# mkln/spamtree

Measured on AMD Instinct MI355X. Metric: Gibbs iterations/sec + achieved HBM GB/s, n=1e6 grid, 1/2/4/8 MI355X, higher is better.
Workload: dtype f64

## Files before the change

### spamtree_amd/csrc/spamtree_fit.cpp

```cpp
#include "spamtree_fit.h"

#include <chrono>
#include <cmath>
#include <cstdlib>
#include <cstring>
#include <string>
#include <vector>

namespace {

struct HostRng {
  uint32_t k0, k1;
  explicit HostRng(uint64_t seed) : k0((uint32_t)seed), k1((uint32_t)(seed >> 32)) {}
  void block(uint32_t c0, uint32_t c1, uint32_t c2, uint32_t c3, uint32_t out[4]) const {
    uint32_t a = k0, b = k1;
    for (int r = 0; r < 10; ++r) {
      const uint64_t p0 = 0xD2511F53ull * c0, p1 = 0xCD9E8D57ull * c2;
      const uint32_t n0 = (uint32_t)(p1 >> 32) ^ c1 ^ a, n2 = (uint32_t)(p0 >> 32) ^ c3 ^ b;
      c1 = (uint32_t)p1; c3 = (uint32_t)p0; c0 = n0; c2 = n2;
      a += 0x9E3779B9u; b += 0xBB67AE85u;
    }
    out[0] = c0; out[1] = c1; out[2] = c2; out[3] = c3;
  }
  static double u01(uint32_t a, uint32_t b) {
// ... 174 lines not shown

extern "C" int stm_init(stm_chain c) {
  if (!c || !c->h) return ST_ERR_USAGE;
  if (c->initialised) return ST_OK;
  for (int slot = 0; slot < 2; ++slot) {
    const int rc = st_factor(c->h, slot, c->param.data(), c->k, &c->loglik[slot]);
    if (rc < 0) { c->err = st_last_error(c->h); return rc; }
    if (rc > 0) { c->err = "starting theta is not positive definite"; return ST_ERR_USAGE; }
  }
  c->current_loglik = c->loglik[0];
  c->initialised = true;
  return ST_OK;
}

static int draw_tausq_beta(stm_chain c);
static int step_w_theta(stm_chain c, bool early_ok = true) {
  const uint32_t m = (uint32_t)c->m;
  int rc;
  const int k = c->k;
  RAMAdapt &am = c->am;
  std::vector<double> U(k), np(k);
  if (c->sample_theta) {
    am.count_proposal();
    for (int i = 0; i < k; ++i) U[i] = c->rng.normal(i, 0, m, 1);
    for (int j = 0; j < k; ++j) {
      double f = logit(c->param[j], c->bounds[j], c->bounds[k + j]);
      for (int i = 0; i < k; ++i) f += am.paramsd[(size_t)i * k + j] * U[i];
      np[j] = logistic(f, c->bounds[j], c->bounds[k + j]);
    }
    for (int j = 0; j < k; ++j) {
      if (np[j] < c->bounds[j]) np[j] = c->bounds[j] + 1e-10;
// ... 14 lines not shown
  };
  if (c->sample_w) {
    rc = st_sample_w_loglik_begin(c->h, nullptr, c->seed, m, 0);
    if (rc) { c->err = st_last_error(c->h); return rc; }
    if ((!c->sample_theta || !c->defer_sync) && (rc = finish_sweep()) != 0) return rc;
    sweep_open = c->sample_theta && c->defer_sync;
  }
  if (c->sample_theta) {
    c->theta_alt = np;
    double new_ll = c->loglik[1];
    if (c->early_beta && early_ok && c->sample_w && st_factor_is_async(c->h)) {
      rc = st_factor_enqueue(c->h, 1, np.data(), k);
      if (rc == 0) {
        const int r3 = draw_tausq_beta(c);
        c->tb_drawn = true;
        rc = st_factor_finish(c->h, &new_ll);
        if (r3) return r3;
      }
    } else
    rc = st_factor(c->h, 1, np.data(), k, &new_ll);
    if (sweep_open) {
      const int r2 = finish_sweep();
      if (r2) return r2;
    }
    if (rc < 0) { c->err = st_last_error(c->h); return rc; }
    const bool acceptable = rc == 0;
    if (acceptable) c->loglik[1] = new_ll;
    c->current_loglik = c->loglik[0];
    if (std::isnan(c->current_loglik)) { c->err = "At nan loglik: error."; return STM_ERR_NAN; }
    double jac = 0;
// ... 54 lines not shown
    if ((rc = st_set_beta(c->h, c->Bcoeff.data())) != 0) { c->err = st_last_error(c->h); return rc; }
  }
  return ST_OK;
}
static int step_tausq_beta(stm_chain c) {
  if (!c->tb_drawn) { const int rc = draw_tausq_beta(c); if (rc) return rc; }
  c->tb_drawn = false;
  c->m += 1;
  return ST_OK;
}

extern "C" int stm_step(stm_chain c, int n_iters) {
  if (!c || !c->h) return ST_ERR_USAGE;
  if (!c->initialised) { const int rc0 = stm_init(c); if (rc0) return rc0; }
  for (int it = 0; it < n_iters; ++it) {
    int rc = step_w_theta(c);
    if (rc) return rc;
    rc = step_tausq_beta(c);
    if (rc) return rc;
  }
  return ST_OK;
}

extern "C" int stm_state(stm_chain c, double *theta, double *Bcoeff, double *tausq_inv, double *loglik, double *accept_ratio,
                         int64_t *iteration, double *paramsd) {
  if (!c) return ST_ERR_USAGE;
  if (theta) std::memcpy(theta, c->param.data(), c->param.size() * sizeof(double));
  if (Bcoeff) std::memcpy(Bcoeff, c->Bcoeff.data(), c->Bcoeff.size() * sizeof(double));
  if (tausq_inv) std::memcpy(tausq_inv, c->tausq_inv.data(), c->tausq_inv.size() * sizeof(double));
  if (loglik) *loglik = c->current_loglik;
  if (accept_ratio) *accept_ratio = c->am.accept_ratio;
// ... 114 lines not shown
```

### spamtree_amd/csrc/spamtree_hip.hip

```cpp

#include "st_device.hpp"
#include "factor_generic.hpp"
#include "factor_mfma.hpp"
#include "chol_blocked.hpp"
#include "factor_quad.hpp"
#include "factor_big.hpp"
#include "factor_wide.hpp"
#include "factor_lchain.hpp"
#include "sample_kernels.hpp"
#include "misc_kernels.hpp"
#include "predict_points.hpp"
#include "simulate_kernels.hpp"

static thread_local std::string g_create_error;
struct st_handle_s;
static void points_free(st_handle_s *h);

template <typename T>
struct DevBuf {
  T *p = nullptr;
  size_t n = 0;
  hipError_t alloc(size_t count) {
    n = count;
    if (count == 0) { p = nullptr; return hipSuccess; }
// ... 59 lines not shown
  "k_factor_mfma", "k_factor_lchain<96>", "k_factor_lchain<136>", "k_factor_ref_finish", "k_lchain_scalars", "k_factor_wide<WG_JT>",
  "k_factor_bigmfma<3, 5, 34>", "k_factor_bigmfma<4, 5, 34>", "k_factor_bigmfma<5, 3, 24>",
  "k_gram", "k_gram_direct", "k_gram_big",
  "k_sample_mfma", "k_sample_leaf_seg<4>", "k_sample_leaf_seg<6>", "k_sample_leaf", "k_sample_wave", "k_sample_lean<true>",
  "k_sample_lean<false>", "k_sample<true, false>", "k_sample_leaf_wide", "k_sample<true, true>", "k_sample<false>",
};

struct Switches {
  int wide = 1, split_gram = 1, sample_wave = 1;
  bool lchain = true, lchain_ref = true, gram_big = true, gram_direct = true, sample_lean = true, sample_lat = true,
       leaf_seg = true, leaf_wide = true, async_top = true;
  int lchain_ref_min = 1;
  int factor_gen = 3;
  int quad_units = 0;
  int quad_min = -1;
};

static Switches read_switches() {
  auto level = [](const char *name) {
    const char *e = getenv(name);
    return (e && e[0] == '0') ? 0 : ((e && e[0] == '2') ? 2 : 1);
  };
  Switches s;
  s.wide = level("SPAMTREE_WIDE"); s.split_gram = level("SPAMTREE_SPLIT_GRAM"); s.sample_wave = level("SPAMTREE_SAMPLE_WAVE");
  s.lchain = level("SPAMTREE_LCHAIN"); s.lchain_ref = level("SPAMTREE_LCHAIN_REF"); s.gram_big = level("SPAMTREE_GRAM_BIG");
  s.gram_direct = level("SPAMTREE_GRAM_DIRECT"); s.sample_lean = level("SPAMTREE_SAMPLE_LEAN"); s.sample_lat = level("SPAMTREE_SAMPLE_LAT");
  s.leaf_seg = level("SPAMTREE_LEAF_SEG"); s.leaf_wide = level("SPAMTREE_LEAF_WIDE"); s.async_top = level("SPAMTREE_ASYNC_TOP");
  const char *e;
  if ((e = getenv("SPAMTREE_LCHAIN_REF_MIN"))) s.lchain_ref_min = atoi(e);
  if ((e = getenv("SPAMTREE_FACTOR_KERNEL")) && e[0] == '1') s.factor_gen = 1;
  if ((e = getenv("SPAMTREE_QUAD_UNITS"))) s.quad_units = atoi(e);
  if ((e = getenv("SPAMTREE_QUAD_MIN"))) s.quad_min = std::max(atoi(e), 0);
  return s;
}

struct st_handle_s {
  std::string err;
  int device = 0;
  hipStream_t stream = nullptr;
  int quirks = 1, force_generic = 0;
  Switches sw;
  long long n_all = 0, n_blocks = 0;
  int q = 1, p = 1, d = 2, n_groups = 0, n_actual_groups = 0;
  long long n_obs = 0;
  size_t lds_limit = 65536;
  int sm_count = 256;

// ... 28 lines not shown
  DevBuf<int> d_ownobs;
  std::vector<int> own_grp_list, own_obs_slow;
  DevBuf<int> d_owngrp, d_ownslow;
  DevBuf<unsigned char> d_rowmask, d_blkmask;
  DevBuf<double> d_comm;
  DevBuf<double> d_gather;
  DevBuf<int> d_gidx;
  int gather_cnt = 1;
  DevBuf<double> d_gerr;
  hipStream_t stream2 = nullptr;
  hipEvent_t ev_top = nullptr, ev_main = nullptr;
  DevBuf<int> d_err2, d_toplist;
  int n_toplist = 0, g_top = 0;
  bool async_top = false, top_pending = false, prof_suspend = false, async_top_off = false;
  hipEvent_t ev_stats = nullptr;
  bool stats_on_stream2 = false;
  bool stats_prefetched = false;
  int top_phys = -1;
  std::vector<double> top_theta;
  long long top_off = 0, top_len = 0;
  std::vector<std::pair<long long, long long>> top_zero;
  bool ext_stream = false;
  DevBuf<double> d_sum_w, d_sum_yhat;
  long long n_summary = 0;
  DevBuf<double> d_draws_w, d_draws_yhat;
  long long draws_cap = 0, n_draws = 0;
  int gram_direct_level = -1;
  bool stats_valid = false;
  bool host_stats_valid = false;
  std::vector<double> host_stats;
  double *pin = nullptr;
  double *pin_up = nullptr;
  int pin_up_slot = 0, pin_up_len = 0;
  hipEvent_t ev_up[2] = {nullptr, nullptr};
  bool factor_open = false; int factor_open_slot = 0;
  std::vector<double> top_theta_open;
  hipEvent_t ev_factor = nullptr;
  std::vector<char> s0_valid;
  bool gram_valid = false;
  bool cache_gram = true;
  bool defer_leaf = false;
  bool leaf_pending[2] = {false, false};
  CovPar leaf_cp[2];
  DevBuf<double> d_vleaf;
  bool limited = false;
  std::vector<int> twin_list;
  DevBuf<int> d_twin;
  int twin_maxM = 1;
  ncclComm_t comm = nullptr;
  std::vector<LevelInfo> levels;
  std::vector<int> route_a, route_b;
  int route_p = R_NONE;
// ... 9 lines not shown
  std::vector<SimLevel> sim_levels;

  DevBuf<double> d_cx, d_cy, d_y, d_X, d_w, d_xb, d_z, d_B, d_panels[2], d_acc, d_logdet[2], d_loglik[2], d_scalars, d_partial,
      d_stats, d_scratch, d_tmp_n, d_tsq;
  DevBuf<int> d_mv, d_anc, d_dch, d_lvl, d_pred, d_allobs, d_err;
  DevBuf<unsigned char> d_obs;
  DevBuf<long long> d_dev2model, d_partner;
  DevBuf<Blk> d_blks;
  size_t panel_total = 0, acc_total = 0;
  long long scratch_stride = 0;
  int scratch_wgs = 0;
  int slot_map[2] = {0, 1};
  double tausq_inv[QMAX];
  std::vector<double> theta[2];
  bool z_valid = false;

  int prof = 0;
  double prof_ms[ST_N_KERNEL_FAMILIES] = {0};
  long long prof_n[ST_N_KERNEL_FAMILIES] = {0};
  std::vector<double> prof_level_ms;
  std::vector<long long> prof_level_n;
  struct ProfRec { hipEvent_t a, b; int fam, level, count; };
  std::vector<ProfRec> prof_pending;
  std::vector<hipEvent_t> ev_free;
};

#define HCHK(h, call)                                                                                         \
  do {                                                                                                        \
    hipError_t e_ = (call);                                                                                   \
    if (e_ != hipSuccess) {                                                                                   \
// ... 77 lines not shown
extern "C" void st_set_create_error(const char *msg) { g_create_error = msg ? msg : ""; }

extern "C" int st_destroy(st_handle h) {
  if (!h) return ST_OK;
  (void)hipSetDevice(h->device);
  h->d_cx.free(); h->d_cy.free(); h->d_y.free(); h->d_X.free(); h->d_w.free(); h->d_xb.free(); h->d_z.free(); h->d_B.free();
  h->d_panels[0].free(); h->d_panels[1].free(); h->d_acc.free();
  for (int s = 0; s < 2; ++s) { h->d_logdet[s].free(); h->d_loglik[s].free(); }
  h->d_scalars.free(); h->d_partial.free(); h->d_stats.free(); h->d_scratch.free(); h->d_tmp_n.free(); h->d_tsq.free();
  h->d_mv.free(); h->d_anc.free(); h->d_dch.free(); h->d_lvl.free(); h->d_pred.free(); h->d_allobs.free(); h->d_err.free();
  h->d_twin.free(); h->d_wgrps.free(); h->d_lcslabs.free(); h->d_lcrow.free(); h->d_rfvoff.free(); h->d_vscr.free(); h->d_vleaf.free(); h->d_s0.free(); h->d_s0off.free(); h->d_obs.free(); h->d_dev2model.free(); h->d_partner.free(); h->d_blks.free(); h->d_grps.free(); h->d_quads.free(); h->d_gdesc.free();
  h->d_ownobs.free(); h->d_owngrp.free(); h->d_ownslow.free(); h->d_rowmask.free(); h->d_blkmask.free(); h->d_comm.free(); h->d_gather.free(); h->d_gidx.free(); h->d_gerr.free(); h->d_err2.free(); h->d_toplist.free();
  if (h->ev_top) (void)hipEventDestroy(h->ev_top);
  if (h->ev_main) (void)hipEventDestroy(h->ev_main);
  if (h->ev_stats) (void)hipEventDestroy(h->ev_stats);
  if (h->stream2) (void)hipStreamDestroy(h->stream2); h->d_sum_w.free(); h->d_sum_yhat.free(); h->d_draws_w.free(); h->d_draws_yhat.free();
  prof_harvest(h);
  for (auto e : h->ev_free) (void)hipEventDestroy(e);
  if (h->comm) (void)ncclCommDestroy(h->comm);
  if (h->pin) (void)hipHostFree(h->pin);
  if (h->pin_up) (void)hipHostFree(h->pin_up);
  for (int i = 0; i < 2; ++i) if (h->ev_up[i]) (void)hipEventDestroy(h->ev_up[i]);
  if (h->ev_factor) (void)hipEventDestroy(h->ev_factor);
  points_free(h);
  h->d_simz.free(); h->d_sime.free(); h->d_simw.free(); h->d_simy.free(); h->d_rowblk.free();
  if (h->stream && !h->ext_stream) (void)hipStreamDestroy(h->stream);
  delete h;
  return ST_OK;
}

static int create_impl(const st_problem *pb, const st_options *opt, st_handle *out, bool plan_only, int64_t *owner_out, int32_t *cut_out);

extern "C" int st_create(const st_problem *pb, const st_options *opt, st_handle *out) {
  return create_impl(pb, opt, out, false, nullptr, nullptr);
}

extern "C" int st_shard_plan(const st_problem *pb, int32_t world, int64_t *owner, int32_t *cut_level) {
  st_options opt = {0, 1, 0, world, 0, 0};
// ... 628 lines not shown
      for (int b2 = 0; b2 < pb->p; ++b2)
        h->xtx[(size_t)v * pb->p * pb->p + (size_t)b2 * pb->p + a] += pb->X[(size_t)a * n + r] * pb->X[(size_t)b2 * n + r];
  }

#define CCHK(call)                                                                                            \
  do {                                                                                                        \
    hipError_t e_ = (call);                                                                                   \
    if (e_ != hipSuccess) return fail_create(h, ST_ERR_HIP, std::string(#call) + ": " + hipGetErrorString(e_)); \
  } while (0)
  CCHK(hipStreamCreate(&h->stream));
  CCHK(hipHostMalloc((void **)&h->pin, 64 * sizeof(double), hipHostMallocDefault));
  h->pin_up_len = QMAX + std::max(1, h->p * h->q);
  CCHK(hipHostMalloc((void **)&h->pin_up, (size_t)2 * h->pin_up_len * sizeof(double), hipHostMallocDefault));
  for (int i = 0; i < 2; ++i) CCHK(hipEventCreateWithFlags(&h->ev_up[i], hipEventDisableTiming));
  CCHK(hipEventCreateWithFlags(&h->ev_factor, hipEventDisableTiming));
  CCHK(h->d_cx.upload(cx)); CCHK(h->d_cy.upload(cy)); CCHK(h->d_y.upload(y)); CCHK(h->d_X.upload(X));
  CCHK(h->d_mv.upload(mv)); CCHK(h->d_obs.upload(obs)); CCHK(h->d_partner.upload(partner));
  CCHK(h->d_dev2model.upload(h->dev2model));
  {
    std::vector<Blk> db = h->blks;
    if (h->limited) for (Blk &B : db) B.acc_len = 0;
    CCHK(h->d_blks.upload(db));
    if (h->limited) { std::vector<int> t = h->twin_list; if (t.empty()) t.push_back(0); CCHK(h->d_twin.upload(t)); }
  }
  { std::vector<int> a = h->anc_idx; if (a.empty()) a.push_back(0); CCHK(h->d_anc.upload(a)); }
  { std::vector<int> a = h->dch_idx; if (a.empty()) a.push_back(0); CCHK(h->d_dch.upload(a)); }
  CCHK(h->d_lvl.upload(h->lvl_list));
  { std::vector<Grp> g = h->grps; if (g.empty()) g.push_back(Grp{0, 0, 0, 0, 0}); CCHK(h->d_grps.upload(g)); }
  {
    int stride = 8;
// ... 214 lines not shown
  {
    h->g_top = 0;
    bool all_fast = !h->limited && !h->force_generic;
    for (int g = 0; g < n_actual; ++g) all_fast = all_fast && h->levels[g].fast;
    if (all_fast) {
      while (h->g_top < n_actual && !(h->sw.factor_gen == 3 && h->levels[h->g_top].q_nkx > 0)) ++h->g_top;
      if (h->g_top >= n_actual) h->g_top = 0;
    }
    h->async_top = h->g_top > 0 && h->sw.async_top;
    std::vector<int> tl;
    for (int b : h->own_obs_list) if (h->blks[b].level < h->g_top) tl.push_back(b);
    h->n_toplist = (int)tl.size();
    if (tl.empty()) tl.push_back(0);
    CCHK(h->d_toplist.upload(tl));
    CCHK(h->d_err2.alloc(2));
    if (h->async_top) {
      CCHK(hipStreamCreateWithFlags(&h->stream2, hipStreamNonBlocking));
      CCHK(hipEventCreateWithFlags(&h->ev_top, hipEventDisableTiming));
      CCHK(hipEventCreateWithFlags(&h->ev_main, hipEventDisableTiming));
      CCHK(hipEventCreateWithFlags(&h->ev_stats, hipEventDisableTiming));
    }
  }
  (void)hipGetLastError();
#undef CCHK
  h->s0_valid.assign((size_t)std::max(n_actual, 1), 0);
  h->prof_level_ms.assign(2 * n_actual, 0.0);
  h->prof_level_n.assign(2 * n_actual, 0);
  *out = h;
  return ST_OK;
}

static int upload_rows(st_handle h, const double *src, double *dst) {
  std::vector<double> tmp(h->n_all);
  for (long long i = 0; i < h->n_all; ++i) tmp[i] = src[h->dev2model[i]];
  HCHK(h, hipMemcpyAsync(dst, tmp.data(), h->n_all * sizeof(double), hipMemcpyHostToDevice, h->stream));
// ... 12 lines not shown
  if (!h || !w) return ST_ERR_USAGE;
  invalidate_stats(h);
  HCHK(h, hipSetDevice(h->device));
  return upload_rows(h, w, h->d_w.p);
}
extern "C" int st_get_w(st_handle h, double *w) {
  if (!h || !w) return ST_ERR_USAGE;
  HCHK(h, hipSetDevice(h->device));
  return download_rows(h, h->d_w.p, w);
}
extern "C" int st_get_xb(st_handle h, double *xb) {
  if (!h || !xb) return ST_ERR_USAGE;
  HCHK(h, hipSetDevice(h->device));
  return download_rows(h, h->d_xb.p, xb);
}
extern "C" int st_set_beta(st_handle h, const double *Bcoeff) {
  if (!h || !Bcoeff) return ST_ERR_USAGE;
  invalidate_stats(h);
  HCHK(h, hipSetDevice(h->device));
  h->pin_up_slot ^= 1;
  HCHK(h, hipEventSynchronize(h->ev_up[h->pin_up_slot]));
  double *stg = h->pin_up + (size_t)h->pin_up_slot * h->pin_up_len + QMAX;
  std::memcpy(stg, Bcoeff, (size_t)h->p * h->q * sizeof(double));
  HCHK(h, hipMemcpyAsync(h->d_B.p, stg, (size_t)h->p * h->q * sizeof(double), hipMemcpyHostToDevice, h->stream));
  HCHK(h, hipEventRecord(h->ev_up[h->pin_up_slot], h->stream));
  {
    ProfScope ps(h, 4);
    const int grid = (int)((h->n_all + NT - 1) / NT);
    hipLaunchKernelGGL(k_xb, dim3(grid), dim3(NT), 0, h->stream, h->d_X.p, h->d_mv.p, h->d_B.p, h->n_all, h->p, h->d_xb.p);
  }
  HCHK(h, hipGetLastError());
  return ST_OK;
}
extern "C" int st_set_tausq_inv(st_handle h, const double *t) {
  if (!h || !t) return ST_ERR_USAGE;
  for (int j = 0; j < h->q; ++j) h->tausq_inv[j] = t[j];
  HCHK(h, hipSetDevice(h->device));
  h->pin_up_slot ^= 1;
  HCHK(h, hipEventSynchronize(h->ev_up[h->pin_up_slot]));
  double *stg = h->pin_up + (size_t)h->pin_up_slot * h->pin_up_len;
  std::memcpy(stg, h->tausq_inv, QMAX * sizeof(double));
  HCHK(h, hipMemcpyAsync(h->d_tsq.p, stg, QMAX * sizeof(double), hipMemcpyHostToDevice, h->stream));
  HCHK(h, hipEventRecord(h->ev_up[h->pin_up_slot], h->stream));
  return ST_OK;
}
static int settle_top(st_handle h) {
  if (h->top_pending) { HCHK(h, hipSetDevice(h->device)); HCHK(h, hipStreamWaitEvent(h->stream, h->ev_top, 0)); }
  return ST_OK;
}
static int complete_leaf(st_handle h, int slot) {
  const int phys = h->slot_map[slot];
  if (!h->leaf_pending[phys]) return ST_OK;
  HCHK(h, hipSetDevice(h->device));
  const CovPar &cp = h->leaf_cp[phys];
  ProfScope phase(h, 0, -2, 0);
  for (int g = 0; g < h->n_actual_groups; ++g) {
    const LevelInfo &L = h->levels[g];
    if (L.vl_off < 0) continue;
    QuadArgs F;
    std::memset(&F, 0, sizeof(F));
    F.blks = h->d_blks.p; F.anc_idx = h->d_anc.p; F.grps = h->d_grps.p + L.grp_first;
    F.quads = h->d_quads.p + L.quad_first + L.qown_lo; F.nquad = L.qown_n;
// ... 202 lines not shown
        hipLaunchKernelGGL((k_factor_wide<WG_JT>), dim3(std::min(L.wide_count, h->sm_count)), dim3(WG_NT), L.lds_wide, st, W, cp);
      } else if (L.bigmfma && h->sw.factor_gen == 3) {
        A.scratch = h->d_scratch.p; A.scratch_stride = h->scratch_stride; A.SR = L.bm_ldS;
        if (L.maxM <= 48) { route(g, R_BIGMFMA3); hipLaunchKernelGGL((k_factor_bigmfma<3, 5, 34>), dim3(std::min(A.nlist, h->sm_count)), dim3(BM_NT), L.lds_bigmfma, st, A, cp); }
        else if (L.maxM <= 64) { route(g, R_BIGMFMA4); hipLaunchKernelGGL((k_factor_bigmfma<4, 5, 34>), dim3(std::min(A.nlist, h->sm_count)), dim3(BM_NT), L.lds_bigmfma, st, A, cp); }
        else { route(g, R_BIGMFMA5); hipLaunchKernelGGL((k_factor_bigmfma<5, 3, 24>), dim3(std::min(A.nlist, h->sm_count)), dim3(BM_NT), L.lds_bigmfma, st, A, cp); }
      } else if (L.big_factor) { route(g, R_FACTOR_SCRATCH); launch_factor<true, MODE_FACTOR>(h, L, A, cp, st); }
      else { route(g, R_FACTOR_LDS); launch_factor<false, MODE_FACTOR>(h, L, A, cp, st); }
    }
    HCHK(h, hipGetLastError());
  }
  return ST_OK;
}


extern "C" int st_factor_ahead_levels(st_handle h) { return (h && h->async_top && !h->async_top_off) ? h->g_top : 0; }
extern "C" int st_factor_ahead_enable(st_handle h, int enable) {
  if (!h) return ST_ERR_USAGE;
  h->async_top_off = !enable;
  return ST_OK;
}
extern "C" int st_factor_begin(st_handle h, int slot, const double *theta, int ntheta) {
  if (!h || !theta || slot < 0 || slot > 1) return ST_ERR_USAGE;
  if (!h->async_top || h->async_top_off) return ST_OK;
  HCHK(h, hipSetDevice(h->device));
  CovPar cp;
  int rc = make_covpar(h, theta, ntheta, &cp);
  if (rc) return rc;
  if (h->top_pending) HCHK(h, hipStreamWaitEvent(h->stream2, h->ev_top, 0));
  HCHK(h, hipEventRecord(h->ev_main, h->stream));
  HCHK(h, hipStreamWaitEvent(h->stream2, h->ev_main, 0));
  const int init[2] = {INT_MAX, 0};
  HCHK(h, hipMemcpyAsync(h->d_err2.p, init, 2 * sizeof(int), hipMemcpyHostToDevice, h->stream2));
  const int phys = h->slot_map[slot];
  h->leaf_pending[phys] = false;
  h->prof_suspend = true;
  rc = factor_launch(h, phys, cp, 0, h->g_top, h->stream2, h->d_err2.p);
  h->prof_suspend = false;
  if (rc) return rc;
  HCHK(h, hipEventRecord(h->ev_top, h->stream2));
  h->top_pending = true; h->top_phys = phys; h->top_theta.assign(theta, theta + ntheta);
  return ST_OK;
}
static int fix_top_comps(st_handle h, int phys);
static int run_stats(st_handle h, hipStream_t st);
static int stats_begin(st_handle h) {
  if (!h->stream2 || h->stats_valid) return ST_OK;
  HCHK(h, hipEventRecord(h->ev_main, h->stream));
  HCHK(h, hipStreamWaitEvent(h->stream2, h->ev_main, 0));
  int rc = run_stats(h, h->stream2);
  if (rc) return rc;
  const size_t nq = (size_t)h->p * h->q + h->q;
  h->stats_prefetched = nq <= 40;
  if (h->stats_prefetched) HCHK(h, hipMemcpyAsync(h->pin + 20, h->d_stats.p, nq * sizeof(double), hipMemcpyDeviceToHost, h->stream2));
  HCHK(h, hipEventRecord(h->ev_stats, h->stream2));
  h->stats_on_stream2 = true;
  return ST_OK;
}

static int factor_local(st_handle h, int slot, const double *theta, int ntheta, bool vonly);
extern "C" int st_factor_local(st_handle h, int slot, const double *theta, int ntheta) { return factor_local(h, slot, theta, ntheta, false); }
static int factor_local(st_handle h, int slot, const double *theta, int ntheta, bool vonly) {
  if (!h || !theta || slot < 0 || slot > 1) return ST_ERR_USAGE;
  HCHK(h, hipSetDevice(h->device));
  CovPar cp;
  int rc = make_covpar(h, theta, ntheta, &cp);
  if (rc) return rc;
  h->theta[slot].assign(theta, theta + ntheta);
  if (slot == 0) { h->gram_valid = false; std::fill(h->s0_valid.begin(), h->s0_valid.end(), 0); }
  rc = reset_err(h);
  if (rc) return rc;
  const int phys = h->slot_map[slot];
  h->leaf_pending[phys] = false;
  if (slot == 1) { rc = stats_begin(h); if (rc) return rc; }
  bool reuse = false;
  if (h->top_pending) {
    HCHK(h, hipStreamWaitEvent(h->stream, h->ev_top, 0));
    reuse = h->top_phys == phys && (int)h->top_theta.size() == ntheta && std::equal(theta, theta + ntheta, h->top_theta.begin());
    h->top_pending = false;
  }
  bool deferred = false;
  rc = factor_launch(h, phys, cp, reuse ? h->g_top : 0, INT_MAX, nullptr, nullptr, vonly, &deferred);
  if (deferred) { h->leaf_pending[phys] = true; h->leaf_cp[phys] = cp; }
  if (rc || !reuse) return rc;
  rc = fix_top_comps(h, phys);
  if (rc) return rc;
  hipLaunchKernelGGL(k_merge_err, dim3(1), dim3(64), 0, h->stream, h->d_err.p, h->d_err2.p);
  HCHK(h, hipGetLastError());
  return ST_OK;
}

extern "C" int st_mg_pack_comps(st_handle h, int slot, void **dev_ptr, int64_t *len) {
  if (!h || slot < 0 || slot > 1) return ST_ERR_USAGE;
  HCHK(h, hipSetDevice(h->device));
  { const int rc0 = settle_top(h); if (rc0) return rc0; }
  const int phys = h->slot_map[slot], nb = (int)h->n_blocks;
  {
    ProfScope ps(h, 3);
    hipLaunchKernelGGL(k_pack_comps, dim3((std::max(nb, h->world) + NT - 1) / NT), dim3(NT), 0, h->stream, h->d_logdet[phys].p,
                       h->d_loglik[phys].p, h->d_blkmask.p, nb, h->d_err.p, h->rank, h->world, h->d_comm.p);
  }
// ... 69 lines not shown
  int rc = factor_enqueue(h, slot, theta, ntheta, false);
  if (rc) return rc;
  return st_factor_finish(h, loglik);
}
extern "C" int st_factor_is_async(st_handle h) { return (h && !(h->world > 1 || h->comm)) ? 1 : 0; }
extern "C" int st_factor_enqueue(st_handle h, int slot, const double *theta, int ntheta) {
  return factor_enqueue(h, slot, theta, ntheta, h && h->defer_leaf && slot == 1);
}
static int factor_enqueue(st_handle h, int slot, const double *theta, int ntheta, bool vonly) {
  if (!h || !theta || slot < 0 || slot > 1) return ST_ERR_USAGE;
  if (h->factor_open) { h->err = "st_factor_enqueue: the previous one has not been finished"; return ST_ERR_USAGE; }
  if (h->world > 1 || h->comm) {
    h->factor_open = true; h->factor_open_slot = slot; h->top_theta_open.assign(theta, theta + ntheta);
    return ST_OK;
  }
  int rc = factor_local(h, slot, theta, ntheta, vonly);
  if (rc) return rc;
  {
    ProfScope ps(h, 3);
    const int phys = h->slot_map[slot];
    launch_sum2(h->stream, h->d_logdet[phys].p, h->d_loglik[phys].p, (int)h->n_blocks, h->d_scalars.p + 8, h->d_scalars.p);
  }
  HCHK(h, hipGetLastError());
  HCHK(h, hipMemcpyAsync(h->pin + 12, h->d_scalars.p, 2 * sizeof(double), hipMemcpyDeviceToHost, h->stream));
  HCHK(h, hipMemcpyAsync(h->pin + 14, h->d_err.p, 2 * sizeof(int), hipMemcpyDeviceToHost, h->stream));
  HCHK(h, hipEventRecord(h->ev_factor, h->stream));
  h->factor_open = true; h->factor_open_slot = slot; h->top_theta_open.clear();
  return ST_OK;
}
extern "C" int st_factor_finish(st_handle h, double *loglik) {
  if (!h) return ST_ERR_USAGE;
  if (!h->factor_open) { h->err = "st_factor_finish without st_factor_enqueue"; return ST_ERR_USAGE; }
  h->factor_open = false;
  if (h->world > 1 || h->comm) {
    if (!h->comm) { h->err = "world > 1: call st_comm_init first, or use st_factor_local / st_mg_pack_comps / (all-reduce) / st_mg_finish"; return ST_ERR_USAGE; }
    int rc = st_factor_local(h, h->factor_open_slot, h->top_theta_open.data(), (int)h->top_theta_open.size());
    if (rc) return rc;
    return exchange_comps_and_finish(h, h->factor_open_slot, loglik);
  }
  HCHK(h, hipSetDevice(h->device));
  HCHK(h, hipEventSynchronize(h->ev_factor));
  const int e0 = ((const int *)(h->pin + 14))[0];
  if (e0 != INT_MAX) return e0 & 15;
  if (loglik) *loglik = h->pin[12] + h->pin[13];
  return ST_OK;
}

static int gather_w_scatter(st_handle h);
extern "C" int st_sample_w_loglik(st_handle h, const double *z, uint64_t seed, uint32_t iter, int slot, double *loglik) {
  if (!h || slot < 0 || slot > 1) return ST_ERR_USAGE;
  { const int rc0 = complete_leaf(h, slot); if (rc0) return rc0; }
  if (h->world > 1 || h->comm) {
    if (!h->comm) {
      int rc = st_sample_w(h, z, seed, iter);
      if (rc) return rc;
// ... 78 lines not shown
  }
  int rc = st_sample_w_local(h, z, seed, iter);
  if (rc) return rc;
  rc = st_sample_w_top(h);
  if (rc) return rc;
  HCHK(h, hipMemcpyAsync(h->pin + 10, h->d_err.p, 2 * sizeof(int), hipMemcpyDeviceToHost, h->stream));
  rc = st_loglik_local(h, slot);
  if (rc) return rc;
  {
    ProfScope ps(h, 3);
    const int phys = h->slot_map[slot];
    launch_sum2(h->stream, h->d_logdet[phys].p, h->d_loglik[phys].p, (int)h->n_blocks, h->d_scalars.p + 8, h->d_scalars.p);
  }
  HCHK(h, hipGetLastError());
  HCHK(h, hipMemcpyAsync(h->pin + 8, h->d_scalars.p, 2 * sizeof(double), hipMemcpyDeviceToHost, h->stream));
  h->c_rc = INT_MIN;
  h->c_pending = true;
  return ST_OK;
}
extern "C" int st_sample_w_loglik_end(st_handle h, double *loglik) {
  if (!h || !h->c_pending) return ST_ERR_USAGE;
  h->c_pending = false;
  if (h->c_rc != INT_MIN) {
    if (h->c_rc == ST_OK && loglik) *loglik = h->c_ll;
    return h->c_rc;
  }
  HCHK(h, hipStreamSynchronize(h->stream));
  const int e0 = ((const int *)(h->pin + 10))[0];
  if (e0 != INT_MAX) return e0 & 15;
  if (loglik) *loglik = h->pin[8] + h->pin[9];
  return ST_OK;
}

static int gen_or_upload_z(st_handle h, const double *z, uint64_t seed, uint32_t iter, unsigned stream_id, double *dst) {
  if (z) return upload_rows(h, z, dst);
  {
    ProfScope ps(h, 5);
    const int grid = (int)((h->n_all + NT - 1) / NT);
    hipLaunchKernelGGL(k_normals, dim3(grid), dim3(NT), 0, h->stream, dst, h->d_dev2model.p, h->n_all, iter, stream_id,
                       (unsigned long long)seed);
  }
  HCHK(h, hipGetLastError());
  return ST_OK;
}

static int sample_launch(st_handle h, int g_hi, int g_lo) {
  const int phys = h->slot_map[0];
  for (int g = g_hi - 1; g >= g_lo; --g) {
    const LevelInfo &L = h->levels[g];
    int *route = h->route_b.data() + 2 * (size_t)g;
    route[0] = route[1] = R_NONE;
    if ((L.fast ? L.gown_n : L.own_n) == 0) continue;
    SampleArgs A;
    std::memset(&A, 0, sizeof(A));
    A.blks = h->d_blks.p; A.anc_idx = h->d_anc.p; A.dch_idx = h->d_dch.p; A.list = h->d_lvl.p + L.first + L.own_lo; A.nlist = L.own_n;
    A.panels = h->d_panels[phys].p; A.w = h->d_w.p; A.y = h->d_y.p; A.xb = h->d_xb.p; A.z = h->d_z.p; A.mv = h->d_mv.p;
    A.obs = h->d_obs.p; A.acc = h->d_acc.p; A.errflag = h->d_err.p; A.maxP = L.maxP; A.maxM = L.maxM; A.maxLd = L.maxLd;
    for (int j = 0; j < QMAX; ++j) A.tausq_inv[j] = h->tausq_inv[j];
    A.do_gram = (h->gram_valid && h->cache_gram) ? 0 : 1;
    A.no_fwd = h->limited ? 1 : 0;
    A.lds_sq = (L.big_sample && L.sample_sq) ? 2 : 0;
    A.s0 = h->d_s0.p; A.s0off = h->d_s0off.p;
    {
// ... 58 lines not shown
        }
        if (L.big_sample) {
          A.scratch = h->d_scratch.p; A.scratch_stride = h->scratch_stride;
          if (L.isref) { route[1] = R_SAMPLE_BIG_REF; hipLaunchKernelGGL((k_sample<true, false>), dim3(std::min(L.own_n, h->scratch_wgs)), dim3(NT), L.lds_sample, h->stream, A); }
          else if (h->sw.leaf_wide && !A.do_gram && L.maxM <= 64 && L.maxMa <= 96 && L.maxJ <= 8) {
            route[1] = R_SAMPLE_LEAF_WIDE;
            hipLaunchKernelGGL(k_sample_leaf_wide, dim3(std::min(L.own_n, 16 * h->sm_count)), dim3(NT), ((size_t)4 * 64 * 12 + 3 * 64) * 8, h->stream, A);
          } else { route[1] = R_SAMPLE_BIG_LEAF; hipLaunchKernelGGL((k_sample<true, true>), dim3(std::min(L.own_n, h->scratch_wgs)), dim3(NT), L.lds_sample, h->stream, A); }
        } else {
          route[1] = R_SAMPLE_SMALL;
          hipLaunchKernelGGL((k_sample<false>), dim3(L.own_n), dim3(NT), L.lds_sample, h->stream, A);
        }
      }
    }
    HCHK(h, hipGetLastError());
  }
  return ST_OK;
}

extern "C" int st_sample_w_local(st_handle h, const double *z, uint64_t seed, uint32_t iter) {
  if (!h) return ST_ERR_USAGE;
  invalidate_stats(h);
  HCHK(h, hipSetDevice(h->device));
  int rc = gen_or_upload_z(h, z, seed, iter, 0u, h->d_z.p);
  if (rc) return rc;
  h->z_valid = true;
  rc = reset_err(h);
  if (rc) return rc;
  rc = sample_launch(h, h->n_actual_groups, std::min(h->cut, h->n_actual_groups));
  if (rc) return rc;
  for (auto &zr : h->top_zero) HCHK(h, hipMemsetAsync(h->d_acc.p + zr.first, 0, (size_t)zr.second * sizeof(double), h->stream));
  return ST_OK;
}
extern "C" int st_mg_top_region(st_handle h, void **dev_ptr, int64_t *len) {
  if (!h) return ST_ERR_USAGE;
  if (dev_ptr) *dev_ptr = h->d_acc.p + h->top_off;
  if (len) *len = h->top_len;
  return ST_OK;
}
extern "C" int st_sample_w_top(st_handle h) {
  if (!h) return ST_ERR_USAGE;
  invalidate_stats(h);
  HCHK(h, hipSetDevice(h->device));
  const int rc = sample_launch(h, std::min(h->cut, h->n_actual_groups), 0);
// ... 115 lines not shown
  }
  HCHK(h, hipGetLastError());
  HCHK(h, reset_err(h) == ST_OK ? hipSuccess : hipErrorUnknown);
  return ST_OK;
}
static int fix_top_comps(st_handle h, int phys) {
  if (h->n_toplist == 0) return ST_OK;
  int maxP = 0, maxM = 0;
  for (int g = 0; g < h->g_top; ++g) { maxP = std::max(maxP, h->levels[g].maxP); maxM = std::max(maxM, h->levels[g].maxM); }
  LoglikArgs A;
  A.blks = h->d_blks.p; A.anc_idx = h->d_anc.p; A.list = h->d_toplist.p; A.nlist = h->n_toplist;
  A.panels = h->d_panels[phys].p; A.w = h->d_w.p; A.loglik_c = h->d_loglik[phys].p; A.maxP = maxP; A.maxM = maxM;
  {
    ProfScope ps(h, 0, h->g_top > 0 ? h->g_top - 1 : 0);
    hipLaunchKernelGGL(k_loglik, dim3(A.nlist), dim3(NT), lds_loglik_bytes(maxP, maxM), h->stream, A);
  }
  HCHK(h, hipGetLastError());
  return ST_OK;
}
extern "C" int st_loglik_w(st_handle h, int slot, double *loglik) {
  if (!h) return ST_ERR_USAGE;
  if (slot >= 0 && slot <= 1) { const int rc0 = complete_leaf(h, slot); if (rc0) return rc0; }
  if (h->world > 1 || h->comm) {
    if (!h->comm) { h->err = "world > 1: call st_comm_init first, or use st_loglik_local / st_mg_pack_comps / (all-reduce) / st_mg_finish"; return ST_ERR_USAGE; }
    int rc = st_loglik_local(h, slot);
    if (rc) return rc;
    return exchange_comps_and_finish(h, slot, loglik);
  }
  int rc = st_loglik_local(h, slot);
  if (rc) return rc;
// ... 807 lines not shown
```

Baseline: 241.6.

## Overlap mid-level factorization on a low-priority stream and prefetch next normals

Extends the async top-level factor path so that the middle reference levels are factored on a third low-priority stream, launched during the sampling sweep after a gate level, with a separate loglik fixup kernel for those groups. The top-level factor launch is deferred until the sampling sweep has started, beta/tau uploads move to the side stream while a factor is open, the next iteration's normals are generated early, and a full stream sync is replaced by an event sync. The aim is to fill idle GPU time between the sweep tail and the factor, at the cost of more streams and events, more complex ordering, and possible contention with the sampling kernels.

```diff
diff --git a/profiles/r05/gaps.py b/profiles/r05/gaps.py
--- /dev/null
+++ b/profiles/r05/gaps.py
@@ -0,0 +1,79 @@
+import argparse
+import csv
+import json
+import statistics
+import sys
+
+
+def load(path):
+    rows = []
+    with open(path, newline="") as f:
+        for r in csv.DictReader(f):
+            rows.append((int(r["Start_Timestamp"]), int(r["End_Timestamp"]), r["Kernel_Name"],
+                         r.get("Queue_Id", "") + "/" + r.get("Stream_Id", "")))
+    rows.sort()
+    return rows
+
+
+def busy_ns(rows, t0, t1):
+    total, cur = 0, t0
+    for s, e, _, _ in rows:
+        if e <= t0 or s >= t1:
+            continue
+        s, e = max(s, cur), min(e, t1)
+        if e > s:
+            total += e - s
+            cur = e
+    return total
+
+
+def main():
+    ap = argparse.ArgumentParser()
+    ap.add_argument("trace")
+    ap.add_argument("--iters", type=int, default=20)
+    ap.add_argument("--gate", type=int, default=2)
+    args = ap.parse_args()
+    rows = load(args.trace)
+    starts = [i for i, r in enumerate(rows) if "k_normals" in r[2]]
+    tails, gaps = [], []
+    for a, b in zip(starts[:-1], starts[1:]):
+        it = rows[a:b]
+        main_q = it[0][3]
+        smp = [r for r in it if "k_sample" in r[2]]
+        llk = [r for r in it if "k_loglik_grp" in r[2]]
+        mrg = [r for r in it if "k_merge_err" in r[2]]
+        if len(smp) <= args.gate or not llk or not mrg:
+            continue
+        t0, t1 = smp[args.gate][1], llk[0][0]
+        other = sum(min(e, t1) - max(s, t0) for s, e, _, q in it if q != main_q and e > t0 and s < t1)
+        tails.append((t1 - t0, busy_ns(rows, t0, t1), other, sum(r[1] - r[0] for r in smp[args.gate + 1:])))
+        quad = [r for r in it if "k_factor_quad" in r[2] and r[0] < mrg[0][0]]
+        nxt = [r for r in rows[b:b + 40] if "k_sample" in r[2]]
+        if not quad or not nxt:
+            continue
+        g0, g1 = quad[-1][1], nxt[0][0]
+        inside = [r for r in rows[a:b + 40] if r[1] > g0 and r[0] < g1]
+        gaps.append((g1 - g0, busy_ns(rows, g0, g1), len(inside), sum(r[1] - r[0] for r in inside)))
+    tails, gaps = tails[-args.iters:], gaps[-args.iters:]
+
+    def med(xs, i):
+        return round(statistics.median(x[i] for x in xs) / 1e3, 1) if xs else None
+
+    span = [rows[s][0] for s in starts][-args.iters - 1:]
+    out = {
+        "iterations": len(tails),
+        "iteration_us": round(statistics.median(b - a for a, b in zip(span[:-1], span[1:])) / 1e3, 1) if len(span) > 1 else None,
+        "tail": {"wall_us": med(tails, 0), "busy_us": med(tails, 1), "idle_us": med(tails, 0) - med(tails, 1) if tails else None,
+                 "other_stream_us": med(tails, 2), "sweep_kernels_us": med(tails, 3)},
+        "gap": {"wall_us": med(gaps, 0), "busy_us": med(gaps, 1), "idle_us": med(gaps, 0) - med(gaps, 1) if gaps else None,
+                "kernels": med(gaps, 2) * 1e3 if gaps else None, "kernel_sum_us": med(gaps, 3)},
+    }
+    if out["tail"]["idle_us"] is not None:
+        out["tail"]["idle_us"] = round(out["tail"]["idle_us"], 1)
+    if out["gap"]["idle_us"] is not None:
+        out["gap"]["idle_us"] = round(out["gap"]["idle_us"], 1)
+    print(json.dumps(out))
+
+
+if __name__ == "__main__":
+    sys.exit(main())
diff --git a/spamtree_amd/csrc/spamtree_fit.cpp b/spamtree_amd/csrc/spamtree_fit.cpp
--- a/spamtree_amd/csrc/spamtree_fit.cpp
+++ b/spamtree_amd/csrc/spamtree_fit.cpp
@@ -212,7 +212,8 @@
 }
 
 static int draw_tausq_beta(stm_chain c);
-static int step_w_theta(stm_chain c, bool early_ok = true) {
+extern "C" int st_normals_begin(st_handle h, uint64_t seed, uint32_t iter);
+static int step_w_theta(stm_chain c, bool early_ok = true, bool more = false) {
   const uint32_t m = (uint32_t)c->m;
   int rc;
   const int k = c->k;
@@ -257,6 +258,10 @@
       if (rc == 0) {
         const int r3 = draw_tausq_beta(c);
         c->tb_drawn = true;
+        if (r3 == 0 && more) {
+          const int r4 = st_normals_begin(c->h, c->seed, m + 1);
+          if (r4) { c->err = st_last_error(c->h); return r4; }
+        }
         rc = st_factor_finish(c->h, &new_ll);
         if (r3) return r3;
       }
@@ -341,7 +346,7 @@
   if (!c || !c->h) return ST_ERR_USAGE;
   if (!c->initialised) { const int rc0 = stm_init(c); if (rc0) return rc0; }
   for (int it = 0; it < n_iters; ++it) {
-    int rc = step_w_theta(c);
+    int rc = step_w_theta(c, true, it + 1 < n_iters);
     if (rc) return rc;
     rc = step_tausq_beta(c);
     if (rc) return rc;
diff --git a/spamtree_amd/csrc/spamtree_hip.hip b/spamtree_amd/csrc/spamtree_hip.hip
--- a/spamtree_amd/csrc/spamtree_hip.hip
+++ b/spamtree_amd/csrc/spamtree_hip.hip
@@ -97,6 +97,8 @@
   int factor_gen = 3;
   int quad_units = 0;
   int quad_min = -1;
+  int async_mid = 1;
+  int mid_gate = 0;
 };
 
 static Switches read_switches() {
@@ -114,6 +116,8 @@
   if ((e = getenv("SPAMTREE_FACTOR_KERNEL")) && e[0] == '1') s.factor_gen = 1;
   if ((e = getenv("SPAMTREE_QUAD_UNITS"))) s.quad_units = atoi(e);
   if ((e = getenv("SPAMTREE_QUAD_MIN"))) s.quad_min = std::max(atoi(e), 0);
+  s.async_mid = level("SPAMTREE_ASYNC_MID");
+  if ((e = getenv("SPAMTREE_MID_GATE"))) s.mid_gate = std::max(atoi(e), 0);
   return s;
 }
 
@@ -172,10 +176,20 @@
   int n_toplist = 0, g_top = 0;
   bool async_top = false, top_pending = false, prof_suspend = false, async_top_off = false;
   hipEvent_t ev_stats = nullptr;
+  hipEvent_t ev_enq = nullptr, ev_up2 = nullptr;
+  bool up_on_stream2 = false;
   bool stats_on_stream2 = false;
   bool stats_prefetched = false;
   int top_phys = -1;
   std::vector<double> top_theta;
+  hipStream_t stream3 = nullptr;
+  hipEvent_t ev_gate = nullptr, ev_mid = nullptr, ev_begin = nullptr;
+  int g_mid = 0, mid_gate_level = 0;
+  bool top_wait = false, top_ahead = false;
+  bool mid_wait = false, mid_ahead = false;
+  CovPar top_cp;
+  DevBuf<int> d_midgrp;
+  int n_midgrp = 0;
   long long top_off = 0, top_len = 0;
   std::vector<std::pair<long long, long long>> top_zero;
   bool ext_stream = false;
@@ -194,6 +208,7 @@
   bool factor_open = false; int factor_open_slot = 0;
   std::vector<double> top_theta_open;
   hipEvent_t ev_factor = nullptr;
+  hipEvent_t ev_c = nullptr;
   std::vector<char> s0_valid;
   bool gram_valid = false;
   bool cache_gram = true;
@@ -233,6 +248,7 @@
   double tausq_inv[QMAX];
   std::vector<double> theta[2];
   bool z_valid = false;
+  bool z_ahead = false; uint64_t z_ahead_seed = 0; uint32_t z_ahead_iter = 0;
 
   int prof = 0;
   double prof_ms[ST_N_KERNEL_FAMILIES] = {0};
@@ -340,6 +356,13 @@
   if (h->ev_top) (void)hipEventDestroy(h->ev_top);
   if (h->ev_main) (void)hipEventDestroy(h->ev_main);
   if (h->ev_stats) (void)hipEventDestroy(h->ev_stats);
+  if (h->ev_gate) (void)hipEventDestroy(h->ev_gate);
+  if (h->ev_begin) (void)hipEventDestroy(h->ev_begin);
+  if (h->ev_enq) (void)hipEventDestroy(h->ev_enq);
+  if (h->ev_up2) (void)hipEventDestroy(h->ev_up2);
+  if (h->ev_mid) (void)hipEventDestroy(h->ev_mid);
+  if (h->stream3) (void)hipStreamDestroy(h->stream3);
+  h->d_midgrp.free();
   if (h->stream2) (void)hipStreamDestroy(h->stream2); h->d_sum_w.free(); h->d_sum_yhat.free(); h->d_draws_w.free(); h->d_draws_yhat.free();
   prof_harvest(h);
   for (auto e : h->ev_free) (void)hipEventDestroy(e);
@@ -348,6 +371,7 @@
   if (h->pin_up) (void)hipHostFree(h->pin_up);
   for (int i = 0; i < 2; ++i) if (h->ev_up[i]) (void)hipEventDestroy(h->ev_up[i]);
   if (h->ev_factor) (void)hipEventDestroy(h->ev_factor);
+  if (h->ev_c) (void)hipEventDestroy(h->ev_c);
   points_free(h);
   h->d_simz.free(); h->d_sime.free(); h->d_simw.free(); h->d_simy.free(); h->d_rowblk.free();
   if (h->stream && !h->ext_stream) (void)hipStreamDestroy(h->stream);
@@ -1006,6 +1030,7 @@
   CCHK(hipHostMalloc((void **)&h->pin_up, (size_t)2 * h->pin_up_len * sizeof(double), hipHostMallocDefault));
   for (int i = 0; i < 2; ++i) CCHK(hipEventCreateWithFlags(&h->ev_up[i], hipEventDisableTiming));
   CCHK(hipEventCreateWithFlags(&h->ev_factor, hipEventDisableTiming));
+  CCHK(hipEventCreateWithFlags(&h->ev_c, hipEventDisableTiming));
   CCHK(h->d_cx.upload(cx)); CCHK(h->d_cy.upload(cy)); CCHK(h->d_y.upload(y)); CCHK(h->d_X.upload(X));
   CCHK(h->d_mv.upload(mv)); CCHK(h->d_obs.upload(obs)); CCHK(h->d_partner.upload(partner));
   CCHK(h->d_dev2model.upload(h->dev2model));
@@ -1250,11 +1275,35 @@
     if (tl.empty()) tl.push_back(0);
     CCHK(h->d_toplist.upload(tl));
     CCHK(h->d_err2.alloc(2));
-    if (h->async_top) {
+    h->g_mid = h->g_top;
+    if (all_fast && h->world == 1 && h->sw.async_mid && h->sw.factor_gen == 3 && (h->g_top == 0 || h->async_top)) {
+      int last_ref = -1;
+      for (int g = 0; g < n_actual; ++g) if (h->levels[g].isref && h->levels[g].count > 0) last_ref = g;
+      while (h->g_mid < last_ref && h->levels[h->g_mid].isref && h->levels[h->g_mid].q_nkx > 0 &&
+             (h->sw.async_mid == 2 || h->levels[h->g_mid].grp_count >= 2 * h->sm_count)) ++h->g_mid;
+    }
+    h->mid_gate_level = std::min(h->g_mid - 1 + h->sw.mid_gate, n_actual - 1);
+    std::vector<int> ml;
+    for (int g = h->g_top; g < h->g_mid; ++g)
+      for (int k = 0; k < h->levels[g].gown_n; ++k) ml.push_back(h->levels[g].grp_first + h->levels[g].gown_lo + k);
+    h->n_midgrp = (int)ml.size();
+    if (ml.empty()) ml.push_back(0);
+    CCHK(h->d_midgrp.upload(ml));
+    if (h->async_top || h->g_mid > h->g_top) {
       CCHK(hipStreamCreateWithFlags(&h->stream2, hipStreamNonBlocking));
       CCHK(hipEventCreateWithFlags(&h->ev_top, hipEventDisableTiming));
       CCHK(hipEventCreateWithFlags(&h->ev_main, hipEventDisableTiming));
+      CCHK(hipEventCreateWithFlags(&h->ev_begin, hipEventDisableTiming));
+      CCHK(hipEventCreateWithFlags(&h->ev_enq, hipEventDisableTiming));
+      CCHK(hipEventCreateWithFlags(&h->ev_up2, hipEventDisableTiming));
       CCHK(hipEventCreateWithFlags(&h->ev_stats, hipEventDisableTiming));
+    }
+    if (h->g_mid > h->g_top) {
+      int prio_least = 0, prio_greatest = 0;
+      CCHK(hipDeviceGetStreamPriorityRange(&prio_least, &prio_greatest));
+      CCHK(hipStreamCreateWithPriority(&h->stream3, hipStreamNonBlocking, prio_least));
+      CCHK(hipEventCreateWithFlags(&h->ev_gate, hipEventDisableTiming));
+      CCHK(hipEventCreateWithFlags(&h->ev_mid, hipEventDisableTiming));
     }
   }
   (void)hipGetLastError();
@@ -1297,6 +1346,16 @@
   HCHK(h, hipSetDevice(h->device));
   return download_rows(h, h->d_xb.p, xb);
 }
+static int upload_stream(st_handle h, hipStream_t *st) {
+  *st = h->stream;
+  if (!(h->factor_open && h->stream2 && h->top_theta_open.empty() && !(h->world > 1 || h->comm))) return ST_OK;
+  if (!h->up_on_stream2) {
+    HCHK(h, hipStreamWaitEvent(h->stream2, h->ev_enq, 0));
+    h->up_on_stream2 = true;
+  }
+  *st = h->stream2;
+  return ST_OK;
+}
 extern "C" int st_set_beta(st_handle h, const double *Bcoeff) {
   if (!h || !Bcoeff) return ST_ERR_USAGE;
   invalidate_stats(h);
@@ -1305,12 +1364,14 @@
   HCHK(h, hipEventSynchronize(h->ev_up[h->pin_up_slot]));
   double *stg = h->pin_up + (size_t)h->pin_up_slot * h->pin_up_len + QMAX;
   std::memcpy(stg, Bcoeff, (size_t)h->p * h->q * sizeof(double));
-  HCHK(h, hipMemcpyAsync(h->d_B.p, stg, (size_t)h->p * h->q * sizeof(double), hipMemcpyHostToDevice, h->stream));
-  HCHK(h, hipEventRecord(h->ev_up[h->pin_up_slot], h->stream));
+  hipStream_t st = nullptr;
+  { const int rc = upload_stream(h, &st); if (rc) return rc; }
+  HCHK(h, hipMemcpyAsync(h->d_B.p, stg, (size_t)h->p * h->q * sizeof(double), hipMemcpyHostToDevice, st));
+  HCHK(h, hipEventRecord(h->ev_up[h->pin_up_slot], st));
   {
-    ProfScope ps(h, 4);
+    ProfScope ps(h, 4, -1, 1, st);
     const int grid = (int)((h->n_all + NT - 1) / NT);
-    hipLaunchKernelGGL(k_xb, dim3(grid), dim3(NT), 0, h->stream, h->d_X.p, h->d_mv.p, h->d_B.p, h->n_all, h->p, h->d_xb.p);
+    hipLaunchKernelGGL(k_xb, dim3(grid), dim3(NT), 0, st, h->d_X.p, h->d_mv.p, h->d_B.p, h->n_all, h->p, h->d_xb.p);
   }
   HCHK(h, hipGetLastError());
   return ST_OK;
@@ -1323,12 +1384,15 @@
   HCHK(h, hipEventSynchronize(h->ev_up[h->pin_up_slot]));
   double *stg = h->pin_up + (size_t)h->pin_up_slot * h->pin_up_len;
   std::memcpy(stg, h->tausq_inv, QMAX * sizeof(double));
-  HCHK(h, hipMemcpyAsync(h->d_tsq.p, stg, QMAX * sizeof(double), hipMemcpyHostToDevice, h->stream));
-  HCHK(h, hipEventRecord(h->ev_up[h->pin_up_slot], h->stream));
+  hipStream_t st = nullptr;
+  { const int rc = upload_stream(h, &st); if (rc) return rc; }
+  HCHK(h, hipMemcpyAsync(h->d_tsq.p, stg, QMAX * sizeof(double), hipMemcpyHostToDevice, st));
+  HCHK(h, hipEventRecord(h->ev_up[h->pin_up_slot], st));
   return ST_OK;
 }
 static int settle_top(st_handle h) {
-  if (h->top_pending) { HCHK(h, hipSetDevice(h->device)); HCHK(h, hipStreamWaitEvent(h->stream, h->ev_top, 0)); }
+  if (h->top_pending && h->top_ahead) { HCHK(h, hipSetDevice(h->device)); HCHK(h, hipStreamWaitEvent(h->stream, h->ev_top, 0)); }
+  if (h->mid_ahead) HCHK(h, hipStreamWaitEvent(h->stream, h->ev_mid, 0));
   return ST_OK;
 }
 static int complete_leaf(st_handle h, int slot) {
@@ -1561,7 +1625,10 @@
 }
 
 
-extern "C" int st_factor_ahead_levels(st_handle h) { return (h && h->async_top && !h->async_top_off) ? h->g_top : 0; }
+extern "C" int st_factor_ahead_levels(st_handle h) {
+  if (!h || h->async_top_off) return 0;
+  return h->g_mid > h->g_top ? h->g_mid : (h->async_top ? h->g_top : 0);
+}
 extern "C" int st_factor_ahead_enable(st_handle h, int enable) {
   if (!h) return ST_ERR_USAGE;
   h->async_top_off = !enable;
@@ -1569,27 +1636,50 @@
 }
 extern "C" int st_factor_begin(st_handle h, int slot, const double *theta, int ntheta) {
   if (!h || !theta || slot < 0 || slot > 1) return ST_ERR_USAGE;
-  if (!h->async_top || h->async_top_off) return ST_OK;
+  const bool has_mid = h->g_mid > h->g_top;
+  if ((!h->async_top && !has_mid) || h->async_top_off) return ST_OK;
   HCHK(h, hipSetDevice(h->device));
   CovPar cp;
   int rc = make_covpar(h, theta, ntheta, &cp);
   if (rc) return rc;
-  if (h->top_pending) HCHK(h, hipStreamWaitEvent(h->stream2, h->ev_top, 0));
-  HCHK(h, hipEventRecord(h->ev_main, h->stream));
-  HCHK(h, hipStreamWaitEvent(h->stream2, h->ev_main, 0));
+  if (h->top_pending && h->top_ahead) HCHK(h, hipStreamWaitEvent(h->stream, h->ev_top, 0));
+  if (h->mid_ahead) HCHK(h, hipStreamWaitEvent(h->stream, h->ev_mid, 0));
+  HCHK(h, hipEventRecord(h->ev_begin, h->stream));
+  const int phys = h->slot_map[slot];
+  h->leaf_pending[phys] = false;
+  h->top_pending = true; h->top_phys = phys; h->top_theta.assign(theta, theta + ntheta); h->top_cp = cp;
+  h->top_wait = true; h->top_ahead = false; h->mid_wait = has_mid; h->mid_ahead = false;
+  return ST_OK;
+}
+static int launch_top(st_handle h) {
+  h->top_wait = false;
+  HCHK(h, hipStreamWaitEvent(h->stream2, h->ev_begin, 0));
   const int init[2] = {INT_MAX, 0};
   HCHK(h, hipMemcpyAsync(h->d_err2.p, init, 2 * sizeof(int), hipMemcpyHostToDevice, h->stream2));
-  const int phys = h->slot_map[slot];
-  h->leaf_pending[phys] = false;
   h->prof_suspend = true;
-  rc = factor_launch(h, phys, cp, 0, h->g_top, h->stream2, h->d_err2.p);
+  const int rc = h->async_top ? factor_launch(h, h->top_phys, h->top_cp, 0, h->g_top, h->stream2, h->d_err2.p) : ST_OK;
   h->prof_suspend = false;
   if (rc) return rc;
   HCHK(h, hipEventRecord(h->ev_top, h->stream2));
-  h->top_pending = true; h->top_phys = phys; h->top_theta.assign(theta, theta + ntheta);
+  h->top_ahead = true;
+  return ST_OK;
+}
+static int launch_mid(st_handle h) {
+  if (h->top_wait) { const int rc0 = launch_top(h); if (rc0) return rc0; }
+  h->mid_wait = false;
+  HCHK(h, hipEventRecord(h->ev_gate, h->stream));
+  HCHK(h, hipStreamWaitEvent(h->stream3, h->ev_gate, 0));
+  HCHK(h, hipStreamWaitEvent(h->stream3, h->ev_top, 0));
+  h->prof_suspend = true;
+  const int rc = factor_launch(h, h->top_phys, h->top_cp, h->g_top, h->g_mid, h->stream3, h->d_err2.p);
+  h->prof_suspend = false;
+  if (rc) return rc;
+  HCHK(h, hipEventRecord(h->ev_mid, h->stream3));
+  h->mid_ahead = true;
   return ST_OK;
 }
 static int fix_top_comps(st_handle h, int phys);
+static int fix_mid_comps(st_handle h, int phys);
 static int run_stats(st_handle h, hipStream_t st);
 static int stats_begin(st_handle h) {
   if (!h->stream2 || h->stats_valid) return ST_OK;
@@ -1620,18 +1710,21 @@
   const int phys = h->slot_map[slot];
   h->leaf_pending[phys] = false;
   if (slot == 1) { rc = stats_begin(h); if (rc) return rc; }
-  bool reuse = false;
+  bool reuse = false, mid = false;
   if (h->top_pending) {
-    HCHK(h, hipStreamWaitEvent(h->stream, h->ev_top, 0));
-    reuse = h->top_phys == phys && (int)h->top_theta.size() == ntheta && std::equal(theta, theta + ntheta, h->top_theta.begin());
-    h->top_pending = false;
+    if (h->top_ahead) HCHK(h, hipStreamWaitEvent(h->stream, h->ev_top, 0));
+    if (h->mid_ahead) HCHK(h, hipStreamWaitEvent(h->stream, h->ev_mid, 0));
+    reuse = h->top_ahead && h->top_phys == phys && (int)h->top_theta.size() == ntheta && std::equal(theta, theta + ntheta, h->top_theta.begin());
+    mid = reuse && h->mid_ahead;
+    h->top_pending = h->top_wait = h->top_ahead = h->mid_wait = h->mid_ahead = false;
   }
   bool deferred = false;
-  rc = factor_launch(h, phys, cp, reuse ? h->g_top : 0, INT_MAX, nullptr, nullptr, vonly, &deferred);
+  rc = factor_launch(h, phys, cp, mid ? h->g_mid : (reuse && h->async_top ? h->g_top : 0), INT_MAX, nullptr, nullptr, vonly, &deferred);
   if (deferred) { h->leaf_pending[phys] = true; h->leaf_cp[phys] = cp; }
   if (rc || !reuse) return rc;
   rc = fix_top_comps(h, phys);
   if (rc) return rc;
+  if (mid) { rc = fix_mid_comps(h, phys); if (rc) return rc; }
   hipLaunchKernelGGL(k_merge_err, dim3(1), dim3(64), 0, h->stream, h->d_err.p, h->d_err2.p);
   HCHK(h, hipGetLastError());
   return ST_OK;
@@ -1731,6 +1824,7 @@
     h->factor_open = true; h->factor_open_slot = slot; h->top_theta_open.assign(theta, theta + ntheta);
     return ST_OK;
   }
+  if (h->stream2) HCHK(h, hipEventRecord(h->ev_enq, h->stream));
   int rc = factor_local(h, slot, theta, ntheta, vonly);
   if (rc) return rc;
   {
@@ -1756,6 +1850,11 @@
     return exchange_comps_and_finish(h, h->factor_open_slot, loglik);
   }
   HCHK(h, hipSetDevice(h->device));
+  if (h->up_on_stream2) {
+    HCHK(h, hipEventRecord(h->ev_up2, h->stream2));
+    HCHK(h, hipStreamWaitEvent(h->stream, h->ev_up2, 0));
+    h->up_on_stream2 = false;
+  }
   HCHK(h, hipEventSynchronize(h->ev_factor));
   const int e0 = ((const int *)(h->pin + 14))[0];
   if (e0 != INT_MAX) return e0 & 15;
@@ -1864,6 +1963,7 @@
   }
   HCHK(h, hipGetLastError());
   HCHK(h, hipMemcpyAsync(h->pin + 8, h->d_scalars.p, 2 * sizeof(double), hipMemcpyDeviceToHost, h->stream));
+  HCHK(h, hipEventRecord(h->ev_c, h->stream));
   h->c_rc = INT_MIN;
   h->c_pending = true;
   return ST_OK;
@@ -1875,7 +1975,7 @@
     if (h->c_rc == ST_OK && loglik) *loglik = h->c_ll;
     return h->c_rc;
   }
-  HCHK(h, hipStreamSynchronize(h->stream));
+  HCHK(h, hipEventSynchronize(h->ev_c));
   const int e0 = ((const int *)(h->pin + 10))[0];
   if (e0 != INT_MAX) return e0 & 15;
   if (loglik) *loglik = h->pin[8] + h->pin[9];
@@ -1883,6 +1983,11 @@
 }
 
 static int gen_or_upload_z(st_handle h, const double *z, uint64_t seed, uint32_t iter, unsigned stream_id, double *dst) {
+  if (dst == h->d_z.p) {
+    const bool have = !z && h->z_ahead && h->z_ahead_seed == seed && h->z_ahead_iter == iter;
+    h->z_ahead = false;
+    if (have) return ST_OK;
+  }
   if (z) return upload_rows(h, z, dst);
   {
     ProfScope ps(h, 5);
@@ -1894,9 +1999,21 @@
   return ST_OK;
 }
 
+extern "C" int st_normals_begin(st_handle h, uint64_t seed, uint32_t iter) {
+  if (!h) return ST_ERR_USAGE;
+  HCHK(h, hipSetDevice(h->device));
+  h->z_ahead = false;
+  const int rc = gen_or_upload_z(h, nullptr, seed, iter, 0u, h->d_z.p);
+  if (rc) return rc;
+  h->z_valid = false;
+  h->z_ahead = true; h->z_ahead_seed = seed; h->z_ahead_iter = iter;
+  return ST_OK;
+}
+
 static int sample_launch(st_handle h, int g_hi, int g_lo) {
   const int phys = h->slot_map[0];
   for (int g = g_hi - 1; g >= g_lo; --g) {
+    if (h->mid_wait && g < h->mid_gate_level) { const int rc = launch_mid(h); if (rc) return rc; }
     const LevelInfo &L = h->levels[g];
     int *route = h->route_b.data() + 2 * (size_t)g;
     route[0] = route[1] = R_NONE;
@@ -1985,6 +2102,7 @@
       }
     }
     HCHK(h, hipGetLastError());
+    if (h->top_wait) { const int rc = launch_top(h); if (rc) return rc; }
   }
   return ST_OK;
 }
@@ -1999,6 +2117,8 @@
   rc = reset_err(h);
   if (rc) return rc;
   rc = sample_launch(h, h->n_actual_groups, std::min(h->cut, h->n_actual_groups));
+  if (rc == ST_OK && h->top_wait) rc = launch_top(h);
+  if (rc == ST_OK && h->mid_wait) rc = launch_mid(h);
   if (rc) return rc;
   for (auto &zr : h->top_zero) HCHK(h, hipMemsetAsync(h->d_acc.p + zr.first, 0, (size_t)zr.second * sizeof(double), h->stream));
   return ST_OK;
@@ -2144,6 +2264,21 @@
   {
     ProfScope ps(h, 0, h->g_top > 0 ? h->g_top - 1 : 0);
     hipLaunchKernelGGL(k_loglik, dim3(A.nlist), dim3(NT), lds_loglik_bytes(maxP, maxM), h->stream, A);
+  }
+  HCHK(h, hipGetLastError());
+  return ST_OK;
+}
+static int fix_mid_comps(st_handle h, int phys) {
+  if (h->n_midgrp == 0) return ST_OK;
+  int maxP = 0;
+  for (auto &L : h->levels) maxP = std::max(maxP, L.maxP);
+  LoglikGrpArgs Gr;
+  Gr.blks = h->d_blks.p; Gr.anc_idx = h->d_anc.p; Gr.grps = h->d_grps.p; Gr.list = h->d_midgrp.p; Gr.nlist = h->n_midgrp;
+  Gr.panels = h->d_panels[phys].p; Gr.w = h->d_w.p; Gr.loglik_c = h->d_loglik[phys].p; Gr.maxP = maxP;
+  Gr.gdesc = h->d_gdesc.p; Gr.gd_stride = h->gd_stride;
+  {
+    ProfScope ps(h, 0, h->g_mid - 1);
+    hipLaunchKernelGGL(k_loglik_grp, dim3(Gr.nlist), dim3(NT), (size_t)(maxP + 32) * sizeof(double), h->stream, Gr);
   }
   HCHK(h, hipGetLastError());
   return ST_OK;
```

New measurement: 241.6. No clear change (-0.0%).
